# Gyeeta/gyeeta

Hardware: AMD Instinct MI355X
Metric: events/sec ingested + p50/p99 quantile error vs reference, 1→8 MI355X (higher is better)
Workload: dtype int64; 1 GPU; C3/C4: 10000 hosts x 1000 services, raw 24-B tcp_ipv4_resp_event_t stream, uniform over services, 1 window (ingest + window close) per step; service_keys_total=10000000, multi_level_windows=0, td_pend_cap=1920, td_pend_cap_is_library_default=False, exchange=none, exchange_requested=none, exchange_fallback=False

## Files before the change

### gyeeta_amd/csrc/gys_engine.hip

```cpp
#include <hip/hip_runtime.h>

#include <algorithm>
#include <array>
#include <atomic>
#include <chrono>
#include <cmath>
#include <cstdarg>
#include <cstdio>
#include <cstdlib>
#include <cstring>
#include <deque>
#include <functional>
#include <map>
#include <memory>
#include <set>
#include <string>
#include <thread>
#include <condition_variable>
#include <mutex>
#include <unordered_map>
#include <unordered_set>
#include <vector>

#include <dlfcn.h>
// ... 663 lines not shown
		fin.list[FIN_CLASS2] = c->merge_list2;
		fin.list[FIN_HUGE] = c->huge_list;
		fin.counts = c->merge_count;
		fin.td_run = c->td_run;
		fin.svc_host = c->svc_host;
		fin.host_spill = c->host_spill;
		fin.counters = c->counters;
		fin.staged_cap = (uint32_t)std::min<uint64_t>(c->staged.cap, 0xFFFFFFFFull);
	}
	if (b.td && c->prespill) {
		fin.td_run0 = c->td_run0;
		fin.td_run1 = c->td_run1;
		fin.td_prevm = c->td_prevm;
		fin.hot = c->pre_hot;
		fin.hot_wr = b.pre ? ((c->pre_seq & 1u) ^ 1u) : (c->pre_seq & 1u);
		fin.append_list = c->append_list;
		fin.append_cap = (uint32_t)c->append_list.cap;
		fin.td_pend = c->td_pend;
		fin.staged = c->staged;
		HIPCHK(hipMemsetAsync(c->merge_count + FIN_APPEND, 0, (FIN_NWORDS - FIN_APPEND) * 4, c->stream));
	}
	if (!b.front.host_local) return GYS_OK;
	RespHostP &hp = b.hp;
	hp.ev = (const uint64_t *)b.d_ev;
	hp.n = b.n;
	hp.segs = b.slot->segs.dev;
	hp.nsegs = b.nsegs;
	hp.hdesc = c->hdesc;
	hp.htbl = c->htbl;
	hp.hlst = c->hlst;
	hp.cand = c->cand_pool;
	hp.hll32 = c->hll32;
	hp.td_cur = c->td_cur;
	hp.td_pend = c->td_pend;
	hp.pcap = c->pcap;
	hp.td_run = c->td_run;
	hp.td_run1 = c->td_run1;
	hp.run_delta = (long long)(((intptr_t)c->staged.p - (intptr_t)c->td_pend.p) / 4);
	hp.staged = c->staged;
	hp.host_spill = c->host_spill;
	hp.spill_stamp = ++c->spill_stamp;
	fin.spill_stamp = hp.spill_stamp;
	hp.fin = fin;
	static const uint32_t dbg = [] { const char *e = getenv("GYS_DBG"); return e ? (uint32_t)atoi(e) : 0u; }();
	hp.dbg = dbg;
	hp.counters = c->counters;
	hp.svc_hll = c->svc_hll;
	hp.svc_hll_p = c->cfg.svc_hll_p;
	hp.ghist = (unsigned long long *)(c->arena + c->al.off_i64sum) + c->al.i64_ghist;
	hp.gmax = (long long *)(c->arena + c->al.off_i64max);
	hp.lds_tbl_entries = b.front.max_tbl;
	hp.lds_key_entries = (uint32_t)align_up(b.front.max_l, 2);
	b.hgrid = b.nsegs;
	return GYS_OK;
}

template <bool SHARED, bool SPILL>
void launch_resp_host_tile(gys_ctx *c, const RespBatch &b)
{
	if (b.tile == 6144u) return launch_resp_host<12, SHARED, SPILL>(c, b.hgrid, b.dyn, b.hp);
	if (b.tile == 16384u) launch_resp_host<16, SHARED, SPILL>(c, b.hgrid, b.dyn, b.hp);
	else launch_resp_host<8, SHARED, SPILL>(c, b.hgrid, b.dyn, b.hp);
}

int resp_launch_host_local(gys_ctx *c, RespBatch &b)
{
	if (b.front.host_split || b.front.host_parts) {
		PinnedPair<gys_resp_seg> &vs = b.slot->vsegs;
		const uint64_t nv = resp_virtual_segments(c->resp_sv.data(), b.nsegs, b.front.host_split, c->cfg.max_hosts, nullptr);
		int rc = vs.grow(nv, (1u << 16) / sizeof(gys_resp_seg));
		if (rc) return rc;
		resp_virtual_segments(c->resp_sv.data(), b.nsegs, b.front.host_split, c->cfg.max_hosts, vs.host);
		HIPCHK(hipMemcpyAsync(vs.dev, vs.host, nv * sizeof(gys_resp_seg), hipMemcpyHostToDevice, c->stream));
		b.hp.segs = vs.dev;
		b.hp.nsegs = b.hgrid = (uint32_t)nv;
	}
	if (b.front.host_split) c->n_batches_host_split++;
	else c->n_batches_host_local++;
	if (b.pre) {
		ProfScope ps(c, "prespill");
		PreSpillP pp{};
		pp.td_cur = c->td_cur;
		pp.td_prevm = c->td_prevm;
		pp.td_run = c->td_run;
		pp.td_run0 = c->td_run0;
		pp.td_run1 = c->td_run1;
		pp.counts = c->merge_count;
		pp.hot = c->pre_hot;
		pp.hot_rd = c->pre_seq & 1u;
		pp.svc_host = c->svc_host;
		pp.host_batch = c->host_batch;
		pp.batch_stamp = c->batch_stamp;
		pp.nsvc = c->nsvc;
		pp.pcap = c->pcap;
		pp.pend_cap = c->pend_cap;
		pp.resv = (unsigned long long *)(c->merge_count + FIN_PRE_RESV);
		pp.run_limit = (uint32_t)std::min<uint64_t>(c->staged.cap - std::min<uint64_t>(b.n, c->staged.cap), 0xFFFFFFFFull);
		++c->pre_seq;
		hipLaunchKernelGGL(k_mark_hosts, dim3((b.nsegs + 255) / 256), dim3(256), 0, c->stream, b.slot->segs.dev, b.nsegs, c->host_batch, c->batch_stamp);
		hipLaunchKernelGGL(k_prespill, dim3((c->nsvc + 255) / 256), dim3(256), 0, c->stream, pp);
	}
	ProfScope ps(c, "resp_host");
	if (b.mode != 0) {
		if (b.front.host_split) launch_resp_host_mode<true, false>(c, b.mode, b.tile == 16384u, b.hgrid, b.dyn, b.hp);
		else launch_resp_host_mode<false, false>(c, b.mode, b.tile == 16384u, b.hgrid, b.dyn, b.hp);
	} else if (b.front.host_split) {
		launch_resp_host_tile<true, false>(c, b);
	} else {
		launch_resp_host_tile<false, false>(c, b);
	}
	return GYS_OK;
}

void resp_launch_pass1(gys_ctx *c, const RespBatch &b)
{
	c->n_batches_general++;
	RespP1 p{};
	p.ev = (const uint64_t *)b.d_ev;
	p.cand = c->cand_pool;
	p.n = b.n;
	p.segs = b.slot->segs.dev;
	p.nsegs = b.nsegs;
	p.lk = c->lk_tbl;
	p.svc_gid = c->svc_gid;
	p.hist_win = c->hist_win;
	p.bitmap = c->bitmap;
	p.hll32 = c->hll32;
	p.cms32 = (uint32_t *)(c->arena + c->al.off_u32) + c->al.u32_cms;
	p.batch_cnt = b.td ? c->batch_cnt : nullptr;
	p.ev_kv = b.td ? c->ev_kv : nullptr;
	p.counters = c->counters;
	p.svc_hll = c->svc_hll;
	p.svc_hll_p = c->cfg.svc_hll_p;
	p.ghist = (unsigned long long *)(c->arena + c->al.off_i64sum) + c->al.i64_ghist;
	p.gmax = (long long *)(c->arena + c->al.off_i64max);
	ProfScope ps(c, "resp_pass1");
	if (b.v6) hipLaunchKernelGGL(k_resp_pass1<true>, dim3(grid_for(b.n, 256, (uint32_t)c->ncu * 8)), dim3(256), 0, c->stream, p);
	else hipLaunchKernelGGL(k_resp_pass1<false>, dim3(grid_for(b.n, 256, (uint32_t)c->ncu * 8)), dim3(256), 0, c->stream, p);
}

void resp_launch_general(gys_ctx *c, const RespBatch &b)
{
	const uint32_t nsvc = c->nsvc, nblk = (nsvc + GYS_SCAN_TILE - 1) / GYS_SCAN_TILE;
	{
		ProfScope ps(c, "scan");
		hipLaunchKernelGGL(k_scan_block_sums, dim3(nblk), dim3(256), 0, c->stream, c->batch_cnt, nsvc, c->scan_block_sums);
		hipLaunchKernelGGL(k_scan_top, dim3(1), dim3(256), 0, c->stream, c->scan_block_sums, nblk);
		hipLaunchKernelGGL(k_scan_final, dim3(nblk), dim3(256), 0, c->stream, c->batch_cnt, nsvc, c->scan_block_sums, c->batch_off);
	}
	{
		ProfScope ps(c, "scatter");
		hipLaunchKernelGGL(k_resp_scatter, dim3(grid_for(b.n, 256, (uint32_t)c->ncu * 8)), dim3(256), 0, c->stream, c->ev_kv, b.n, c->batch_off, c->staged);
	}
	ProfScope ps(c, "key_append");
	AppendP ap{};
	ap.batch_cnt = c->batch_cnt;
	ap.off_end = c->batch_off;
	ap.staged = c->staged;
	ap.td_cur = c->td_cur;
	ap.td_pend = c->td_pend;
	ap.pcap = c->pcap;
	ap.nsvc = nsvc;
	const uint32_t nchunks = (nsvc + 63u) / 64u;
	hipLaunchKernelGGL(k_key_append, dim3(std::min<uint32_t>((nchunks + 3u) / 4u, (uint32_t)c->ncu * 8)), dim3(256), 0, c->stream, ap);
}

void resp_launch_finalize(gys_ctx *c, RespBatch &b)
{
	const bool host_local = b.front.host_local;
	if (!host_local || b.front.host_split) {
		ProfScope ps(c, "key_finalize");
		b.fin.batch_off = host_local ? nullptr : c->batch_off;
		hipLaunchKernelGGL(k_key_finalize, dim3((c->nsvc + 255) / 256), dim3(256), 0, c->stream, b.fin);
	}
	if (b.pre)
		hipLaunchKernelGGL(k_run_append, dim3((uint32_t)c->ncu), dim3(256), 0, c->stream, c->append_list, c->merge_count + FIN_APPEND, c->staged, c->td_pend, c->pcap);
	if (host_local && b.n > (uint64_t)c->pcap - c->pend_cap) {
		ProfScope ps(c, "resp_spill");
		if (b.mode != 0) launch_resp_host_mode<true, true>(c, b.mode, b.tile == 16384u, b.hgrid, b.dyn, b.hp);
		else launch_resp_host_tile<true, true>(c, b);
	}
}

void resp_launch_slow_pass(gys_ctx *c, const DigestP &d, uint32_t cap, int top)
{
	MergeP mp{};
	mp.d = d;
	mp.list = c->merge_list_slow;
	mp.count = c->merge_count + FIN_SLOW;
	const dim3 grid(std::max(1u, std::min<uint32_t>(cap, (uint32_t)c->ncu)));
	if (top == 2) hipLaunchKernelGGL((k_digest_merge<GYS_MERGE_LDS_MAX, 1024u>), grid, dim3(1024), 0, c->stream, mp);
	else if (top == 0 && c->merge_fast <= GYS_MERGE_CLASS0) hipLaunchKernelGGL((k_digest_merge<GYS_MERGE_CLASS0, 256u>), grid, dim3(256), 0, c->stream, mp);
	else hipLaunchKernelGGL((k_digest_merge<GYS_MERGE_CLASS1, 256u>), grid, dim3(256), 0, c->stream, mp);
}

void resp_launch_merges(gys_ctx *c, const RespBatch &b)
{
	const uint32_t nsvc = c->nsvc, ncu = (uint32_t)c->ncu;
	const uint32_t cap = (uint32_t)std::min<uint64_t>(nsvc, b.n);
	const bool reach[3] = {true, c->merge_fast < GYS_MERGE_CLASS1 && b.n > c->merge_fast - c->pend_cap, b.n > GYS_MERGE_CLASS1 - c->pend_cap};
	const int top = reach[2] ? 2 : reach[1] ? 1 : 0;
	MergeEnt *const lists[3] = {c->merge_list, c->merge_list1, c->merge_list2};
	MergeBP bp{};
	bp.d = digest_params(c);
	bp.slow_list = c->merge_list_slow;
	bp.slow_count = c->merge_count + FIN_SLOW;
	for (int cls = 0; cls < 3; ++cls) {
		if (!reach[cls]) continue;
		ProfScope ps(c, cls ? "digest_merge_big" : "digest_merge");
		bp.list = lists[cls];
		bp.count = c->merge_count + FIN_CLASS0 + cls;
		if (cls == 0) {
			const dim3 bgrid(std::max(1u, std::min<uint32_t>(cap, ncu * 8)));
			if (c->merge_fast <= 1024u) hipLaunchKernelGGL((k_digest_bins<false, 4u>), bgrid, dim3(256), 0, c->stream, bp);
			else if (c->merge_fast <= 2048u) hipLaunchKernelGGL((k_digest_bins<false, 8u>), bgrid, dim3(256), 0, c->stream, bp);
			else hipLaunchKernelGGL((k_digest_bins<false, 16u>), bgrid, dim3(256), 0, c->stream, bp);
		} else if (cls == 1) {
			hipLaunchKernelGGL((k_digest_bins<false, 16u>), dim3(std::max(1u, std::min<uint32_t>(cap, ncu * GYS_MB_WAVES16))), dim3(256), 0, c->stream, bp);
		} else {
			const uint32_t cap2 = (uint32_t)std::min<uint64_t>(nsvc, b.n / (GYS_MERGE_CLASS1 - c->pend_cap) + 1);
			hipLaunchKernelGGL((k_digest_bins<false, 64u>), dim3(std::max(1u, std::min<uint32_t>(cap2, ncu * 8))), dim3(256), 0, c->stream, bp);
		}
		if (cls == top) resp_launch_slow_pass(c, bp.d, cap, top);
	}
}

void resp_launch_huge(gys_ctx *c, const RespBatch &b)
{
	ProfScope ps(c, "digest_huge");
	Huge2P q{};
	q.d = digest_params(c);
// ... 3161 lines not shown
} GYS_CATCH_ALL

int gys_export_svc_counters(gys_ctx *c, uint32_t first_slot, uint32_t nslots, uint64_t *out)
try {
	GYS_ENTER(c);
	RANGE_CHECK(first_slot, nslots);
	{
		const int rcf = conn_fold(c);
		if (rcf) return rcf;
	}
	HIPCHK(hipMemcpyAsync(out, c->svc_ctr + (size_t)first_slot * 4, (size_t)nslots * 32, hipMemcpyDeviceToHost, c->stream));
	HIPCHK(hipStreamSynchronize(c->stream));
	return GYS_OK;
} GYS_CATCH_ALL

int gys_export_svc_hll(gys_ctx *c, uint32_t first_slot, uint32_t nslots, uint8_t *out)
try {
	GYS_ENTER(c);
	RANGE_CHECK(first_slot, nslots);
	if (!c->svc_hll) return GYS_ERR_STATE;
	HIPCHK(hipMemcpyAsync(out, c->svc_hll + ((size_t)first_slot << c->cfg.svc_hll_p), (size_t)nslots << c->cfg.svc_hll_p, hipMemcpyDeviceToHost, c->stream));
	HIPCHK(hipStreamSynchronize(c->stream));
	return GYS_OK;
} GYS_CATCH_ALL

int gys_export_svc_hll_level(gys_ctx *c, int level, uint64_t tusec, uint32_t first_slot, uint32_t nslots, uint8_t *out)
try {
	GYS_ENTER(c);
	RANGE_CHECK(first_slot, nslots);
	HLL_LEVEL_CHECK(level);
	if (!nslots) return GYS_OK;
	DevBuf<uint8_t> tmp;
	int rc = tmp.grow((size_t)nslots << c->cfg.svc_hll_p, c->stream);
	if (rc == GYS_OK) rc = hll_level_view(c, level, tusec, first_slot, nslots, tmp.p, nullptr);
	if (rc) return rc;
	HIPCHK(hipMemcpyAsync(out, tmp.p, (size_t)nslots << c->cfg.svc_hll_p, hipMemcpyDeviceToHost, c->stream));
	HIPCHK(hipStreamSynchronize(c->stream));
	return GYS_OK;
} GYS_CATCH_ALL

int gys_get_counters(gys_ctx *c, gys_counters *out)
try {
	GYS_ENTER(c);
	if (!c || !out) return GYS_ERR_INVAL;
	uint64_t v[32];
	static_assert(CTR_NUM <= 31, "counter block (the last word is the sink of k_read_events)");
	HIPCHK(hipMemcpyAsync(v, c->counters, sizeof(v), hipMemcpyDeviceToHost, c->stream));
	HIPCHK(hipStreamSynchronize(c->stream));
#ifdef GYS_RESP_TIMING
	{
		unsigned long long t[16];
		HIPCHK(hipMemcpyFromSymbol(t, HIP_SYMBOL(gys::g_resp_timing), sizeof(t)));
		unsigned long long tot = 0;
		for (int i = 0; i < 12; ++i) tot += t[i];
		static const char *nm[12] = {"loads", "probe2", "probe3+", "kept/atomics", "ghist+hash", "hllq/store", "barrier1", "scan1+b", "scan2+b", "image+b", "prologue", "flush"};
		fprintf(stderr, "GYS_RESP_TIMING waves %llu ticks %llu:", t[15], tot);
		for (int i = 0; i < 12; ++i) fprintf(stderr, " %s %.1f%%", nm[i], tot ? 100.0 * (double)t[i] / (double)tot : 0.0);
		fprintf(stderr, "\n");
	}
#endif
#ifdef GYS_HUGE_TIMING
	fprintf(stderr, "GYS_HUGE_TIMING ticks: load %llu words+tail %llu scan %llu assign %llu writeback %llu | entries %llu npend %llu nc %llu\n", (unsigned long long)v[20], (unsigned long long)v[21], (unsigned long long)v[22], (unsigned long long)v[23], (unsigned long long)v[24], (unsigned long long)v[25], (unsigned long long)v[26], (unsigned long long)v[27]);
#endif
	out->resp_events = v[CTR_RESP_EVENTS];
	out->resp_dropped_range = v[CTR_RESP_DROP_RANGE];
	out->resp_dropped_nolistener = v[CTR_RESP_DROP_NOLISTENER];
	out->conn_events = v[CTR_CONN_EVENTS];
	out->conn_unknown_service = v[CTR_CONN_UNKNOWN];
	out->conn_new = v[CTR_CONN_NEW];
	out->conn_closed = v[CTR_CONN_CLOSED];
	out->conn_closed_no_notify = v[CTR_CONN_CLOSED_NO_NOTIFY];
	out->conn_client_side = v[CTR_CONN_CLI_SIDE];
	out->resp_run_overflow = v[CTR_RESP_RUN_OVERFLOW];
	out->lstate_records = v[CTR_LSTATE_RECORDS];
	out->lstate_missed = v[CTR_LSTATE_MISSED];
	out->lstate_errors = v[CTR_LSTATE_ERRORS];
	out->lstate_deleted = v[CTR_LSTATE_DELETED];
	out->resp_batches_host_local = c->n_batches_host_local;
	out->resp_batches_general = c->n_batches_general;
	out->window_graph_launches = c->win_graph_launches;
	out->resp_batches_host_split = c->n_batches_host_split;
	out->td_merges = v[CTR_TD_MERGES];
	out->td_merge_values = v[CTR_TD_MERGE_VALUES];
	out->actconn_records = v[CTR_ACTCONN_RECORDS];
	out->actconn_remote_listen = v[CTR_ACTCONN_REMOTE_LISTEN];
	out->actconn_unknown_listener = v[CTR_ACTCONN_UNKNOWN];
	out->stage_waits = c->ring.waits.load();
	auto snap = [](SubQ &q, uint64_t *calls, uint64_t *submissions) {
		std::lock_guard<std::mutex> g(q.mu);
		*calls = q.calls;
		*submissions = q.submissions;
		return q.tail_flushes;
	};
	out->resp_tail_flushes = snap(c->sq[SubQ::RESP], &out->resp_calls_queued, &out->resp_submissions);
	out->rec_tail_flushes = snap(c->sq[SubQ::CONN], &out->conn_calls_queued, &out->conn_submissions);
	out->rec_tail_flushes += snap(c->sq[SubQ::LSTATE], &out->lstate_calls_queued, &out->lstate_submissions);
	return GYS_OK;
} GYS_CATCH_ALL

int gys_resp_queue_pending(gys_ctx *c, uint64_t *events)
try {
	if (!c || !events) return GYS_ERR_INVAL;
	SubQ &q = c->sq[SubQ::RESP];
	std::lock_guard<std::mutex> g(q.mu);
	uint64_t n = 0;
	if (q.open >= 0) n += q.b[q.open].fill;
	for (int bi : q.sealed) n += q.b[bi].fill;
	*events = n;
	return GYS_OK;
} GYS_CATCH_ALL

// ... 374 lines not shown
```

### gyeeta_amd/csrc/gys_kernels.hpp

```cpp
#pragma once

#include "gys_device.hpp"

namespace gys {

#define GYS_HUGE_VALUE_BITS 20
#define GYS_HUGE_BINS (1u << GYS_HUGE_VALUE_BITS)
#define GYS_ROW_BITS 6
#define GYS_ROW_MASK 0x3Fu
#define GYS_ROW_V6 0x20u
#define GYS_BM_WORDS 32u
#define GYS_STAGED_WORD(tresp, cli_port) ((uint64_t)(((uint32_t)(tresp) << GYS_ROW_BITS) | ((uint32_t)(cli_port) & 0x1Fu)))
#define GYS_STAGED_WORD_FAM(tresp, cli_port, v6) ((uint32_t)(((uint32_t)(tresp) << GYS_ROW_BITS) | ((v6) ? GYS_ROW_V6 : 0u) | ((uint32_t)(cli_port) & 0x1Fu)))

enum { CTR_RESP_EVENTS = 0, CTR_RESP_DROP_RANGE, CTR_RESP_DROP_NOLISTENER, CTR_CONN_EVENTS, CTR_CONN_UNKNOWN, CTR_LSTATE_RECORDS,
       CTR_LSTATE_MISSED, CTR_LSTATE_ERRORS, CTR_LSTATE_DELETED, CTR_TD_MERGES, CTR_TD_MERGE_VALUES, CTR_ACTCONN_RECORDS, CTR_ACTCONN_REMOTE_LISTEN, CTR_ACTCONN_UNKNOWN,
       CTR_CONN_NEW, CTR_CONN_CLOSED, CTR_CONN_CLOSED_NO_NOTIFY, CTR_CONN_CLI_SIDE, CTR_RESP_RUN_OVERFLOW, CTR_NUM };

__global__ void k_table_set(DevTable t, const uint64_t *kv, uint32_t n)
{
	const uint32_t i = blockIdx.x * blockDim.x + threadIdx.x;
	if (i >= n) return;
	const uint64_t key = kv[2u * i];
	uint32_t h = get_uint64_hash(key) & t.mask;
// ... 313 lines not shown
	const uint64_t stride = (uint64_t)gridDim.x * blockDim.x;
	for (uint64_t i = (uint64_t)blockIdx.x * blockDim.x + threadIdx.x; i < n; i += stride) {
		const uint64_t kv = ev_kv[i];
		if (kv == ~0ull) continue;
		const uint32_t pos = atomicAdd(&off[(uint32_t)(kv >> 32)], 1u);
		staged[pos] = (uint32_t)kv;
	}
}

struct TdMeta {
	uint32_t npend;
	uint16_t nh;
	uint16_t nw;
	uint32_t win_epoch;
	uint32_t hw_epoch;
};
static_assert(sizeof(TdMeta) == 16, "TdMeta is read and written as one 16-byte word");
static_assert(GYS_TD_PEND_CAP == GYS_TDIGEST_PEND_CAP, "gysketch.h and gys_tdigest_tbl.h disagree on the t-digest buffer size");
static_assert(GYS_TD_NB == GYS_TDIGEST_NB && GYS_TD_NB <= 256, "the merge kernels hold one cluster per thread of a 256-thread group");

#define GYS_SPILL_BIT 0x80000000u
#define GYS_RESPILL_BIT 0x40000000u
#define GYS_MERGE_LDS_MAX 16384u
#define GYS_PCAP_MAX 16384u

struct MergeEnt {
	uint32_t slot;
	uint32_t nbuf;
	uint32_t mrun;
	uint32_t off_end;
};

__global__ void k_minmax_init(int2 *mm, uint64_t n)
{
	for (uint64_t i = (uint64_t)blockIdx.x * blockDim.x + threadIdx.x; i < n; i += (uint64_t)gridDim.x * blockDim.x) mm[i] = make_int2(INT32_MAX, INT32_MIN);
}

#define GYS_MERGE_CLASS0 1024u
#define GYS_MERGE_CLASS1 4096u
static_assert(GYS_TDIGEST_MERGE_FAST == GYS_MERGE_CLASS0, "the early re-clustering rule keeps a key's merges inside merge size class 0 (default buffer size)");
enum {
	FIN_CLASS0 = 0, FIN_CLASS1, FIN_CLASS2,
	FIN_HUGE,
	FIN_RUN_ALLOC,
	FIN_SLOW,
	FIN_HUGE_FB,
	FIN_HUGE_NENT,
	FIN_BATCH_CLEARED,
	FIN_QUERY_ONE = FIN_BATCH_CLEARED,
	FIN_HUGE_TAIL,
	FIN_HUGE_TB,
	FIN_APPEND = 12,
	FIN_PRE_RESV = 14,
	FIN_NWORDS = 16
};

struct FinP {
	uint32_t *td_cur;
	TdMeta *td_meta;
	uint32_t nsvc, pcap, epoch;
	uint32_t pend_cap, merge_fast;
	uint32_t *resp_win;
	MergeEnt *list[4];
	uint32_t *counts;
	uint32_t *td_run;
	const uint32_t *batch_off;
	const uint32_t *svc_host;
	uint32_t *host_spill;
	uint32_t spill_stamp;
	uint64_t *counters;
	const uint32_t *td_run0, *td_run1;
	uint32_t *td_prevm, *hot;
	uint32_t hot_wr;
	MergeEnt *append_list;
	uint32_t class2_max;
	uint32_t append_cap;
	uint32_t staged_cap;
	uint32_t *td_pend;
	const uint32_t *staged;
};

template <bool WRITE_CUR>
__device__ __forceinline__ int finalize_one(const FinP &p, bool valid, uint32_t key, uint32_t cur, MergeEnt &ent)
{
	int cls = -1;
	ent = MergeEnt{};
	if (valid) {
		const uint4 mraw = *(const uint4 *)&p.td_meta[key];
		const uint32_t npend0 = mraw.x;
		const bool pre = (cur & GYS_SPILL_BIT) != 0u;
		uint32_t run0 = 0;
		bool run_ok = false;
		if (pre) {
			run0 = p.td_run0[key];
			const uint32_t fill = p.td_run[key];
			run_ok = fill <= p.td_run1[key];
			cur = npend0 + (fill - run0);
			if (fill == run0) {
				p.td_cur[key] = npend0;
				p.td_prevm[key] = 0u;
			}
		}
		if (cur != npend0) {
			const uint32_t m = cur - npend0;
			uint32_t nh = mraw.y & 0xFFFFu, nw = mraw.y >> 16, win_epoch = mraw.z;
			if (win_epoch != p.epoch) {
				nw = npend0;
// ... 259 lines not shown
}

struct HostDesc {
	uint32_t tbl_off;
	uint32_t mask;
	uint32_t nlst;
	uint32_t lst_off;
	uint32_t part;
	uint32_t pmask;
	uint32_t cand_off;
	uint32_t pad;
};

#define GYS_HOST_TBL_EMPTY 0xFFFFFFFFFFFFFFFFull
#define GYS_EV_DROPPED 0xFFFFFFFFu
#define GYS_HOST_THREADS 1024
#define GYS_RESP_THREADS(TPT) ((TPT) == 12 ? 512 : 1024)
#define GYS_SPLIT_PART 65536u

#ifdef GYS_RESP_TIMING
__device__ unsigned long long g_resp_timing[16];
#define GYS_TICK(i) do { const unsigned long long t_now__ = (unsigned long long)clock64(); tacc[i] += (uint32_t)(t_now__ - t_prev__); t_prev__ = t_now__; } while (0)
#else
#define GYS_TICK(i) do { } while (0)
#endif
struct RespHostP {
	const uint64_t *ev;
	uint64_t n;
	const gys_resp_seg *segs;
	uint32_t nsegs;
	const HostDesc *hdesc;
	const uint64_t *htbl;
	const uint32_t *hlst;
	const ListenerCand *cand;
	uint32_t *hll32;
	uint32_t *td_cur;
	uint32_t *td_pend;
	uint32_t pcap;
	uint32_t *td_run;
	const uint32_t *td_run1;
	long long run_delta;
	uint32_t *staged;
	const uint32_t *host_spill;
	uint32_t spill_stamp;
	uint64_t *counters;
	uint8_t *svc_hll;
	uint32_t svc_hll_p;
	unsigned long long *ghist;
	long long *gmax;
	uint32_t lds_tbl_entries;
	uint32_t lds_key_entries;
	FinP fin;
	uint32_t dbg;
};

__host__ __device__ __forceinline__ size_t resp_host_lds_bytes(uint32_t tbl_entries, uint32_t key_entries, uint32_t tile)
{
	return ((size_t)tbl_entries + 2u) * 8u + (size_t)key_entries * 24u + ((size_t)tile + 2u) * 6u;
}

#ifndef GYS_RESP_DBG
#define GYS_RESP_DBG 0
#endif
#define GYS_GH_STRIDE 17u
#define GYS_HQ_CAP 512u
#define GYS_DST_BIAS 65536ull
#ifndef GYS_OPAQUE_LOADED4
#define GYS_OPAQUE_LOADED4(a) asm volatile("" : "+v"(a[0]), "+v"(a[1]), "+v"(a[2]), "+v"(a[3]))
#endif
#define GYS_MEM_FENCE() asm volatile("" ::: "memory")

template <uint32_t T>
__host__ __device__ __forceinline__ uint32_t resp_slot_stride(uint32_t r)
{
	return r >= 4u * T ? T : (((r + 3u) / 4u + 63u) & ~63u);
}

template <int TPT, bool SHARED, bool SPILL, bool SVCHLL, int MODE = 0>
__global__ __launch_bounds__(GYS_RESP_THREADS(TPT), 4) void k_resp_host(RespHostP p_arg)
{
#if defined(__HIP_DEVICE_COMPILE__)
	typedef const RespHostP __attribute__((address_space(4))) *KernargP;
	KernargP p_k = (KernargP)__builtin_amdgcn_kernarg_segment_ptr();
#define GYS_RESP_P_RELOAD() asm volatile("" : "+s"(p_k))
	const RespHostP &p = *(const RespHostP *)p_k;
#else
#define GYS_RESP_P_RELOAD() (void)0
	const RespHostP &p = p_arg;
#endif
	constexpr uint32_t T = GYS_RESP_THREADS(TPT);
	constexpr uint32_t TILE = (uint32_t)TPT * T;
	constexpr bool DBG = GYS_RESP_DBG != 0;
	constexpr bool V6 = MODE == 2;
	constexpr uint32_t SW = V6 ? GYS_EV6_WORDS : 3u;
	GYS_DYN_LDS(uint64_t, s_dyn);
	__shared__ uint32_t s_wsum[T / 64];
	__shared__ uint32_t s_drop[2];
	__shared__ uint32_t s_floor[2];
	__shared__ uint32_t s_fqm[4];
	__shared__ unsigned long long s_gh[16 * GYS_GH_STRIDE];
	__shared__ int32_t s_gmax;
	__shared__ uint32_t s_bk[256];
	__shared__ uint32_t s_hq[SPILL ? 1 : GYS_HQ_CAP];
	__shared__ uint32_t s_hqn;
	__shared__ FinWg s_fin;
	__shared__ uint32_t s_park[64];
	if (!SPILL) resp_bucket_lut_init(s_bk, threadIdx.x, T);
	const uint32_t Lc = p.lds_key_entries;
	uint64_t *s_tbl = s_dyn;
	uint64_t *s_dst = s_dyn + p.lds_tbl_entries + 2u;
	uint32_t *s_cur = (uint32_t *)(s_dst + Lc);
	uint32_t *s_slot = s_cur + Lc;
	uint32_t *s_ts2 = s_slot + Lc;
	uint32_t *s_val = s_ts2 + 2u * Lc;
	uint16_t *s_key = (uint16_t *)(s_val + TILE + 2u);
	const uint32_t tid = threadIdx.x, lane = tid & 63u, wave = tid >> 6;
	const gys_resp_seg seg = p.segs[blockIdx.x];
	const uint64_t e0 = seg.first_event;
	uint32_t nx = blockIdx.x + 1;
	if (seg.reserved)
		while (nx < p.nsegs && p.segs[nx].reserved && p.segs[nx].host_slot == seg.host_slot && p.segs[nx].first_event == e0) ++nx;
	uint64_t e1 = nx < p.nsegs ? p.segs[nx].first_event : p.n;
	if (e1 > p.n) e1 = p.n;
	if (e1 <= e0) return;
	if (SPILL && p.host_spill[seg.host_slot] != p.spill_stamp) return;
	const HostDesc hd = p.hdesc[seg.reserved ? seg.reserved - 1u : seg.host_slot];
	const uint32_t mask = hd.mask, L = hd.nlst;
	for (uint32_t i = tid; i <= mask; i += T) s_tbl[i] = p.htbl[hd.tbl_off + i];
	for (uint32_t k = tid; k < L; k += T) {
		const uint32_t slot = p.hlst[hd.lst_off + k];
		const uint32_t c = p.td_cur[slot];
		s_slot[k] = slot;
		s_cur[k] = SPILL ? (c & GYS_RESPILL_BIT) : c;
		s_ts2[k] = 0;
		s_ts2[Lc + k] = 0;
	}
	if (tid < 2) s_drop[tid] = 0;
	if (tid < 16u * GYS_GH_STRIDE) s_gh[tid] = 0;
	if (tid == 0) {
		s_hqn = 0;
		s_floor[0] = SPILL ? 0u : 0xFFFFFFFFu;
		s_floor[1] = 0xFFFFFFFFu;
		s_gmax = INT32_MIN;
		s_tbl[mask + 1u] = p.htbl[hd.tbl_off];
		s_val[TILE] = 0;
		s_key[TILE] = 0;
	}
	__syncthreads();
	if (!SPILL) {
		if (e1 - e0 >= 4096u) {
			uint32_t mn = 0xFFFFFFFFu;
			const uint4 *h4 = (const uint4 *)p.hll32;
			for (uint32_t i = tid; i < (1u << GYS_HLL_P) / 4u; i += T) {
				const uint4 v = h4[i];
				mn = min(min(mn, min(v.x, v.y)), min(v.z, v.w));
			}
			mn = wave_min_u32(mn);
			if (lane == 0) atomicMin(&s_floor[0], mn);
		} else if (tid == 0) {
			s_floor[0] = 0;
		}
		__syncthreads();
		if (tid == 0) s_floor[1] = s_floor[0];
		if (tid < 4) s_fqm[tid] = s_floor[0];
	}
	uint32_t hll_floor = 0;
	const uint32_t K = (L + T - 1) / T;
	const uint32_t klo = min(L, tid * K), khi = min(L, klo + K);
	uint32_t *const dst = SPILL ? p.staged : p.td_pend;
	uint32_t *const dstb = dst - GYS_DST_BIAS;

	uint32_t ndrop_range = 0, ndrop_nol = 0, tile_no = 0, dbg_sink = 0;
#ifdef GYS_RESP_TIMING
	uint32_t tacc[16] = {0, 0, 0, 0, 0, 0, 0, 0, 0, 0, 0, 0, 0, 0, 0, 0};
	unsigned long long t_prev__ = (unsigned long long)clock64();
#endif
	const uint32_t tid24 = 24u * tid;
	const uint32_t wbase = (uint32_t)__builtin_amdgcn_readfirstlane((int)(tid & ~63u));
	int32_t tmax = INT32_MIN, wmax = -1;
	GYS_TICK(10);
	for (uint64_t t0 = e0; t0 < e1; t0 += TILE, ++tile_no) {
		GYS_RESP_P_RELOAD();
		uint32_t *const s_ts = s_ts2 + (tile_no & 1u) * Lc;
#if GYS_PARK_INDEX
#if defined(__HIP_DEVICE_COMPILE__)
		typedef uint32_t park_ix_t;
#else
		typedef ptrdiff_t park_ix_t;
#endif
		const park_ix_t park_ix = (park_ix_t)(&s_park[lane] - s_ts);
#endif
		if (!SPILL) hll_floor = (uint32_t)__builtin_amdgcn_readfirstlane((int)s_floor[tile_no & 1u]);
		const uint64_t left = e1 - t0;
		const uint32_t rem = (uint32_t)__builtin_amdgcn_readfirstlane((int)(left < (uint64_t)TILE ? (uint32_t)left : TILE));
		const uint64_t *const tb = p.ev + (uint64_t)SW * t0;
		uint32_t wd[TPT], lr[TPT];
#pragma unroll
		for (int u = 0; u < TPT; ++u) {
			wd[u] = GYS_EV_DROPPED;
			lr[u] = 0;
		}
#pragma unroll 1
		for (int g = 0; g < TPT; g += 4) {
			if ((uint32_t)g * T >= rem) break;
			const uint32_t S = resp_slot_stride<T>(rem - (uint32_t)g * T);
			if (wbase >= S) break;
			uint64_t w0[4], w1[4], w2[4];
			bool in[4];
#pragma unroll
			for (int u = 0; u < 4; ++u) {
				const uint32_t first = (uint32_t)g * T + (uint32_t)u * S, last = min(rem, first + S);
				const uint32_t ob_raw = tid24 + 24u * first;
				in[u] = ob_raw < 24u * last;
				const uint32_t ob = in[u] ? ob_raw : 0u;
				if (V6) {
					static_assert(GYS_EV6_WORDS == 6, "ob = 24 o: word 6 o of the tile is ob / 4");
					w0[u] = 0;
					w1[u] = tb[ob / 4u + 4u];
					w2[u] = tb[ob / 4u + 5u];
				} else {
					const char *const tbb = (const char *)tb;
					w0[u] = *(const uint64_t *)(tbb + ob);
					w1[u] = *(const uint64_t *)(tbb + ob + 8u);
					w2[u] = *(const uint64_t *)(tbb + ob + 16u);
				}
			}
			GYS_OPAQUE_LOADED4(w0);
			GYS_OPAQUE_LOADED4(w1);
			GYS_OPAQUE_LOADED4(w2);
			GYS_TICK(0);
			uint32_t tresp[4], local[4];
			uint64_t ea[4], eb[4];
// ... 294 lines not shown
				s_key[pos] = (uint16_t)(lr[u] & 0xFFFu);
			}
		}
		__syncthreads();
		GYS_TICK(9);
		if (!SPILL && hq_cur < (hq_e >> 16)) atomicMax(&p.hll32[hq_e & 0xFFFFu], hq_e >> 16);
		{
			uint32_t ntile = 0;
#pragma unroll
			for (uint32_t w = 0; w < T / 64; ++w) ntile += s_wsum[w];
			if (DBG && (p.dbg & 3u)) ntile = 0;
			constexpr int FU = 8;
			constexpr uint32_t NQ = (1u << GYS_HLL_P) / 16u / T;
			uint4 fq[NQ];
			const bool fq_on = !SPILL && t0 + 2ull * TILE < e1;
			if (fq_on) {
#pragma unroll
				for (uint32_t j = 0; j < NQ; ++j) fq[j] = ((const uint4 *)p.hll32)[(tile_no & 3u) * ((1u << GYS_HLL_P) / 16u) + j * T + tid];
			}
			for (uint32_t eb0 = 0; eb0 < ntile; eb0 += (uint32_t)FU * T) {
				uint32_t kk[FU], vv[FU];
				uint64_t dd[FU];
#pragma unroll
				for (int j = 0; j < FU; ++j) {
					const uint32_t e = eb0 + (uint32_t)j * T + tid;
					const uint32_t ee = e < ntile ? e : TILE;
					kk[j] = s_key[ee];
					vv[j] = s_val[ee];
				}
				GYS_MEM_FENCE();
#pragma unroll
				for (int j = 0; j < FU; ++j) dd[j] = s_dst[kk[j]];
				GYS_MEM_FENCE();
#pragma unroll
				for (int j = 0; j < FU; ++j) {
					const uint32_t e = eb0 + (uint32_t)j * T + tid;
					if (e < ntile && dd[j]) dstb[dd[j] + e] = vv[j];
				}
			}
			if (fq_on) {
				uint32_t mn = 0xFFFFFFFFu;
#pragma unroll
				for (uint32_t j = 0; j < NQ; ++j) mn = min(min(mn, min(fq[j].x, fq[j].y)), min(fq[j].z, fq[j].w));
				mn = wave_min_u32(mn);
				if (lane == 0) {
					const uint32_t qn = tile_no & 3u;
					atomicMin(&s_fqm[qn], mn);
					atomicMin(&s_floor[tile_no & 1u], min(min(mn, s_fqm[(qn + 1u) & 3u]), min(s_fqm[(qn + 2u) & 3u], s_fqm[(qn + 3u) & 3u])));
				}
			}
		}
		GYS_TICK(11);
	}
#ifdef GYS_RESP_TIMING
	if (!SPILL && lane == 0) {
#pragma unroll
		for (int i = 0; i < 12; ++i) atomicAdd(&g_resp_timing[i], (unsigned long long)tacc[i]);
		atomicAdd(&g_resp_timing[15], 1ull);
	}
#endif
	if (SPILL) return;
	if (DBG && dbg_sink == 0xDEADBEEFu) p.counters[CTR_RESP_EVENTS] = 1;
	if (wmax >= 0) tmax = wmax >> GYS_ROW_BITS;
	tmax = wave_max_i32(tmax);
	if (lane == 0 && tmax != INT32_MIN) atomicMax(&s_gmax, tmax);
	if (ndrop_range) atomicAdd(&s_drop[0], ndrop_range);
	if (ndrop_nol) atomicAdd(&s_drop[1], ndrop_nol);
	__syncthreads();
	if (tid < 64u) {
		unsigned long long cnt = 0, sum = 0;
		if (tid < 15u) {
			for (uint32_t w = 0; w < 16u; ++w) {
				const unsigned long long v = s_gh[w * GYS_GH_STRIDE + tid];
				cnt += v >> 40;
				sum += v & ((1ull << 40) - 1);
			}
			if (cnt) {
				atomicAdd(&p.ghist[2 * tid], cnt);
				atomicAdd(&p.ghist[2 * tid + 1], sum);
			}
		}
		unsigned long long tot = cnt;
#pragma unroll
		for (int d = 8; d >= 1; d >>= 1) tot += (unsigned long long)__shfl_xor((long long)tot, d, 64);
		if (tid == 0 && tot) atomicAdd(&p.ghist[30], tot);
	}
	if (!SHARED) {
		constexpr int KMAX = (int)(2048u / T);
		bool fvalid[KMAX];
		uint32_t fkey[KMAX], fcur[KMAX];
#pragma unroll
		for (int j = 0; j < KMAX; ++j) {
			const uint32_t k = (uint32_t)j * T + tid;
			fvalid[j] = k < L;
			fkey[j] = fvalid[j] ? s_slot[k] : 0u;
			fcur[j] = fvalid[j] ? s_cur[k] : 0u;
		}
		finalize_keys_wg<true, KMAX>(p.fin, &s_fin, tid, lane, fvalid, fkey, fcur);
	}
	if (tid == 0) {
		if (s_gmax != INT32_MIN) atomicMax(p.gmax, (long long)s_gmax);
		if (hd.part == 0u) atomicAdd((unsigned long long *)&p.counters[CTR_RESP_EVENTS], (unsigned long long)(e1 - e0));
		if (s_drop[0]) atomicAdd((unsigned long long *)&p.counters[CTR_RESP_DROP_RANGE], (unsigned long long)s_drop[0]);
		if (s_drop[1]) atomicAdd((unsigned long long *)&p.counters[CTR_RESP_DROP_NOLISTENER], (unsigned long long)s_drop[1]);
	}
}

struct AppendP {
	uint32_t *batch_cnt;
	const uint32_t *off_end;
	const uint32_t *staged;
	uint32_t *td_cur;
	uint32_t *td_pend;
	uint32_t pcap, nsvc;
};

__global__ __launch_bounds__(256) void k_key_append(AppendP p)
{
	const uint32_t lane = threadIdx.x & 63u;
	const uint32_t nchunks = (p.nsvc + 63u) / 64u, nwaves = gridDim.x * 4u;
	for (uint32_t chunk = blockIdx.x * 4u + (threadIdx.x >> 6); chunk < nchunks; chunk += nwaves) {
		const uint32_t key = chunk * 64u + lane;
		const uint32_t m = key < p.nsvc ? p.batch_cnt[key] : 0u;
		unsigned long long todo = __ballot(m != 0);
		if (!todo) continue;
		const uint32_t oend = m ? p.off_end[key] : 0u;
		const uint32_t cur = m ? p.td_cur[key] : 0u;
		if (m) {
			p.batch_cnt[key] = 0;
			p.td_cur[key] = cur + m;
		}
		while (todo) {
			const int k = __ffsll((long long)todo) - 1;
			todo &= todo - 1;
			const uint32_t km = (uint32_t)__shfl((int)m, k, 64), ke = (uint32_t)__shfl((int)oend, k, 64), kc = (uint32_t)__shfl((int)cur, k, 64);
			if ((uint64_t)kc + km > (uint64_t)p.pcap) continue;
			const uint32_t *src = p.staged + (ke - km);
			uint32_t *dst = p.td_pend + (size_t)(chunk * 64u + (uint32_t)k) * p.pcap + kc;
			for (uint32_t i = lane; i < km; i += 64u) dst[i] = src[i];
		}
	}
}

struct DigestP {
	int64_t *td_sum;
	uint32_t *td_cnt;
	TdMeta *td_meta;
	int2 *td_minmax;
	uint32_t *td_pend;
	uint32_t *td_cur;
	uint32_t pcap, nsvc;
	uint32_t pend_cap;
	const uint32_t *staged;
	gys_hist_rec *hist_win, *hist_all;
	uint32_t *bitmap;
};

#define GYS_WAVE_SYNC()                                              \
// ... 2907 lines not shown
```

Before: 76.89 billion events/s.

## Convert resp_host kernel to a persistent grid with an atomic segment work queue

The per-host response kernel now launches at most one workgroup per CU (two for the 6144 tile). Each workgroup loops over segments, taking the next one from an atomic counter that is cleared before launch. Per-workgroup setup (LDS stats, drop counters, ghist, gmax) and the final flush to global counters run once per workgroup rather than once per segment. The HLL floor scan is also cached across segments. This removes launch and prologue/epilogue cost for very many small segments, but fewer resident workgroups may lower occupancy, and the stale HLL floor plus reliance on the counter reset add risk. The spill pass keeps the old one-workgroup-per-segment grid.

```diff
diff --git a/gyeeta_amd/csrc/gys_engine.hip b/gyeeta_amd/csrc/gys_engine.hip
--- a/gyeeta_amd/csrc/gys_engine.hip
+++ b/gyeeta_amd/csrc/gys_engine.hip
@@ -739,7 +739,14 @@
 	hp.lds_tbl_entries = b.front.max_tbl;
 	hp.lds_key_entries = (uint32_t)align_up(b.front.max_l, 2);
 	b.hgrid = b.nsegs;
-	return GYS_OK;
+	if (!c->prespill) HIPCHK(hipMemsetAsync(c->merge_count + FIN_RESP_WORK, 0, 4, c->stream));
+	return GYS_OK;
+}
+
+void resp_persistent_grid(gys_ctx *c, RespBatch &b)
+{
+	b.hgrid = std::min<uint32_t>(b.hp.nsegs, (uint32_t)c->ncu * (b.tile == 6144u ? 2u : 1u));
+	b.hp.work = c->merge_count + FIN_RESP_WORK;
 }
 
 template <bool SHARED, bool SPILL>
@@ -787,6 +794,7 @@
 		hipLaunchKernelGGL(k_mark_hosts, dim3((b.nsegs + 255) / 256), dim3(256), 0, c->stream, b.slot->segs.dev, b.nsegs, c->host_batch, c->batch_stamp);
 		hipLaunchKernelGGL(k_prespill, dim3((c->nsvc + 255) / 256), dim3(256), 0, c->stream, pp);
 	}
+	resp_persistent_grid(c, b);
 	ProfScope ps(c, "resp_host");
 	if (b.mode != 0) {
 		if (b.front.host_split) launch_resp_host_mode<true, false>(c, b.mode, b.tile == 16384u, b.hgrid, b.dyn, b.hp);
@@ -864,6 +872,8 @@
 		hipLaunchKernelGGL(k_run_append, dim3((uint32_t)c->ncu), dim3(256), 0, c->stream, c->append_list, c->merge_count + FIN_APPEND, c->staged, c->td_pend, c->pcap);
 	if (host_local && b.n > (uint64_t)c->pcap - c->pend_cap) {
 		ProfScope ps(c, "resp_spill");
+		b.hgrid = b.hp.nsegs;
+		b.hp.work = nullptr;
 		if (b.mode != 0) launch_resp_host_mode<true, true>(c, b.mode, b.tile == 16384u, b.hgrid, b.dyn, b.hp);
 		else launch_resp_host_tile<true, true>(c, b);
 	}
@@ -4131,11 +4141,11 @@
 		unsigned long long t[16];
 		HIPCHK(hipMemcpyFromSymbol(t, HIP_SYMBOL(gys::g_resp_timing), sizeof(t)));
 		unsigned long long tot = 0;
-		for (int i = 0; i < 12; ++i) tot += t[i];
-		static const char *nm[12] = {"loads", "probe2", "probe3+", "kept/atomics", "ghist+hash", "hllq/store", "barrier1", "scan1+b", "scan2+b", "image+b", "prologue", "flush"};
+		for (int i = 0; i < 13; ++i) tot += t[i];
+		static const char *nm[13] = {"loads", "probe2", "probe3+", "kept/atomics", "ghist+hash", "hllq/store", "barrier1", "scan1+b", "scan2+b", "image+b", "prologue", "flush", "epilogue"};
 		fprintf(stderr, "GYS_RESP_TIMING waves %llu ticks %llu:", t[15], tot);
-		for (int i = 0; i < 12; ++i) fprintf(stderr, " %s %.1f%%", nm[i], tot ? 100.0 * (double)t[i] / (double)tot : 0.0);
-		fprintf(stderr, "\n");
+		for (int i = 0; i < 13; ++i) fprintf(stderr, " %s %.1f%%", nm[i], tot ? 100.0 * (double)t[i] / (double)tot : 0.0);
+		fprintf(stderr, " | workgroups %llu resident %.3f ms in all (ncu %d)\n", t[14], (double)t[13] / 1e5, c->ncu);
 	}
 #endif
 #ifdef GYS_HUGE_TIMING
diff --git a/gyeeta_amd/csrc/gys_kernels.hpp b/gyeeta_amd/csrc/gys_kernels.hpp
--- a/gyeeta_amd/csrc/gys_kernels.hpp
+++ b/gyeeta_amd/csrc/gys_kernels.hpp
@@ -389,7 +389,8 @@
 	FIN_HUGE_TB,
 	FIN_APPEND = 12,
 	FIN_PRE_RESV = 14,
-	FIN_NWORDS = 16
+	FIN_RESP_WORK = 16,
+	FIN_NWORDS = 17
 };
 
 struct FinP {
@@ -755,6 +756,7 @@
 	uint32_t lds_key_entries;
 	FinP fin;
 	uint32_t dbg;
+	uint32_t *work;
 };
 
 __host__ __device__ __forceinline__ size_t resp_host_lds_bytes(uint32_t tbl_entries, uint32_t key_entries, uint32_t tile)
@@ -785,7 +787,7 @@
 #if defined(__HIP_DEVICE_COMPILE__)
 	typedef const RespHostP __attribute__((address_space(4))) *KernargP;
 	KernargP p_k = (KernargP)__builtin_amdgcn_kernarg_segment_ptr();
-#define GYS_RESP_P_RELOAD() asm volatile("" : "+s"(p_k))
+#define GYS_RESP_P_RELOAD() do { p_k = (KernargP)__builtin_amdgcn_kernarg_segment_ptr(); asm volatile("" : "+s"(p_k)); } while (0)
 	const RespHostP &p = *(const RespHostP *)p_k;
 #else
 #define GYS_RESP_P_RELOAD() (void)0
@@ -808,6 +810,14 @@
 	__shared__ uint32_t s_hqn;
 	__shared__ FinWg s_fin;
 	__shared__ uint32_t s_park[64];
+	__shared__ uint32_t s_next;
+	__shared__ uint32_t s_fl_ok;
+	__shared__ unsigned long long s_nev;
+#ifdef GYS_RESP_TIMING
+	const unsigned long long wg_t0__ = (unsigned long long)wall_clock64();
+	uint32_t tacc[16] = {0, 0, 0, 0, 0, 0, 0, 0, 0, 0, 0, 0, 0, 0, 0, 0};
+	unsigned long long t_prev__ = (unsigned long long)clock64();
+#endif
 	if (!SPILL) resp_bucket_lut_init(s_bk, threadIdx.x, T);
 	const uint32_t Lc = p.lds_key_entries;
 	uint64_t *s_tbl = s_dyn;
@@ -818,19 +828,44 @@
 	uint32_t *s_val = s_ts2 + 2u * Lc;
 	uint16_t *s_key = (uint16_t *)(s_val + TILE + 2u);
 	const uint32_t tid = threadIdx.x, lane = tid & 63u, wave = tid >> 6;
-	const gys_resp_seg seg = p.segs[blockIdx.x];
+	if (tid < 2) s_drop[tid] = 0;
+	if (tid < 16u * GYS_GH_STRIDE) s_gh[tid] = 0;
+	if (tid == 0) {
+		s_gmax = INT32_MIN;
+		s_fl_ok = 0;
+		s_nev = 0;
+	}
+	uint32_t hll_floor = 0;
+	uint32_t *const dst = SPILL ? p.staged : p.td_pend;
+	uint32_t *const dstb = dst - GYS_DST_BIAS;
+	uint32_t ndrop_range = 0, ndrop_nol = 0, tile_no = 0, dbg_sink = 0;
+	const uint32_t tid24 = 24u * tid;
+	const uint32_t wbase = (uint32_t)__builtin_amdgcn_readfirstlane((int)(tid & ~63u));
+	int32_t tmax = INT32_MIN, wmax = -1;
+	uint32_t sg = blockIdx.x;
+	while (sg < p.nsegs) {
+	uint32_t ptid = tid;
+	GYS_OPAQUE_VGPR(ptid);
+	uint32_t nxt = 0;
+	if (ptid == 0) nxt = p.work ? gridDim.x + atomicAdd(p.work, 1u) : sg + gridDim.x;
+	const gys_resp_seg seg = p.segs[sg];
 	const uint64_t e0 = seg.first_event;
-	uint32_t nx = blockIdx.x + 1;
+	uint32_t nx = sg + 1;
 	if (seg.reserved)
 		while (nx < p.nsegs && p.segs[nx].reserved && p.segs[nx].host_slot == seg.host_slot && p.segs[nx].first_event == e0) ++nx;
 	uint64_t e1 = nx < p.nsegs ? p.segs[nx].first_event : p.n;
 	if (e1 > p.n) e1 = p.n;
-	if (e1 <= e0) return;
-	if (SPILL && p.host_spill[seg.host_slot] != p.spill_stamp) return;
+	if (e1 <= e0 || (SPILL && p.host_spill[seg.host_slot] != p.spill_stamp)) {
+		__syncthreads();
+		if (ptid == 0) s_next = nxt;
+		__syncthreads();
+		sg = (uint32_t)__builtin_amdgcn_readfirstlane((int)s_next);
+		continue;
+	}
 	const HostDesc hd = p.hdesc[seg.reserved ? seg.reserved - 1u : seg.host_slot];
 	const uint32_t mask = hd.mask, L = hd.nlst;
-	for (uint32_t i = tid; i <= mask; i += T) s_tbl[i] = p.htbl[hd.tbl_off + i];
-	for (uint32_t k = tid; k < L; k += T) {
+	for (uint32_t i = ptid; i <= mask; i += T) s_tbl[i] = p.htbl[hd.tbl_off + i];
+	for (uint32_t k = ptid; k < L; k += T) {
 		const uint32_t slot = p.hlst[hd.lst_off + k];
 		const uint32_t c = p.td_cur[slot];
 		s_slot[k] = slot;
@@ -838,49 +873,44 @@
 		s_ts2[k] = 0;
 		s_ts2[Lc + k] = 0;
 	}
-	if (tid < 2) s_drop[tid] = 0;
-	if (tid < 16u * GYS_GH_STRIDE) s_gh[tid] = 0;
-	if (tid == 0) {
+	if (ptid == 0) {
 		s_hqn = 0;
-		s_floor[0] = SPILL ? 0u : 0xFFFFFFFFu;
-		s_floor[1] = 0xFFFFFFFFu;
-		s_gmax = INT32_MIN;
+		if (SPILL || !s_fl_ok) {
+			s_floor[0] = SPILL ? 0u : 0xFFFFFFFFu;
+			s_floor[1] = 0xFFFFFFFFu;
+		}
 		s_tbl[mask + 1u] = p.htbl[hd.tbl_off];
 		s_val[TILE] = 0;
 		s_key[TILE] = 0;
 	}
 	__syncthreads();
-	if (!SPILL) {
+	if (ptid == 0) {
+		s_next = nxt;
+		if (!SPILL && hd.part == 0u) s_nev += e1 - e0;
+	}
+	if (!SPILL && !__builtin_amdgcn_readfirstlane((int)s_fl_ok)) {
 		if (e1 - e0 >= 4096u) {
 			uint32_t mn = 0xFFFFFFFFu;
 			const uint4 *h4 = (const uint4 *)p.hll32;
-			for (uint32_t i = tid; i < (1u << GYS_HLL_P) / 4u; i += T) {
+			for (uint32_t i = ptid; i < (1u << GYS_HLL_P) / 4u; i += T) {
 				const uint4 v = h4[i];
 				mn = min(min(mn, min(v.x, v.y)), min(v.z, v.w));
 			}
 			mn = wave_min_u32(mn);
-			if (lane == 0) atomicMin(&s_floor[0], mn);
-		} else if (tid == 0) {
+			if ((ptid & 63u) == 0) {
+				atomicMin(&s_floor[0], mn);
+				atomicMin(&s_floor[1], mn);
+			}
+		} else if (ptid == 0) {
 			s_floor[0] = 0;
+			s_floor[1] = 0;
 		}
 		__syncthreads();
-		if (tid == 0) s_floor[1] = s_floor[0];
-		if (tid < 4) s_fqm[tid] = s_floor[0];
-	}
-	uint32_t hll_floor = 0;
+		if (ptid < 4) s_fqm[ptid] = s_floor[0];
+		if (ptid == 0 && e1 - e0 >= 4096u) s_fl_ok = 1;
+	}
 	const uint32_t K = (L + T - 1) / T;
 	const uint32_t klo = min(L, tid * K), khi = min(L, klo + K);
-	uint32_t *const dst = SPILL ? p.staged : p.td_pend;
-	uint32_t *const dstb = dst - GYS_DST_BIAS;
-
-	uint32_t ndrop_range = 0, ndrop_nol = 0, tile_no = 0, dbg_sink = 0;
-#ifdef GYS_RESP_TIMING
-	uint32_t tacc[16] = {0, 0, 0, 0, 0, 0, 0, 0, 0, 0, 0, 0, 0, 0, 0, 0};
-	unsigned long long t_prev__ = (unsigned long long)clock64();
-#endif
-	const uint32_t tid24 = 24u * tid;
-	const uint32_t wbase = (uint32_t)__builtin_amdgcn_readfirstlane((int)(tid & ~63u));
-	int32_t tmax = INT32_MIN, wmax = -1;
 	GYS_TICK(10);
 	for (uint64_t t0 = e0; t0 < e1; t0 += TILE, ++tile_no) {
 		GYS_RESP_P_RELOAD();
@@ -1281,15 +1311,29 @@
 		}
 		GYS_TICK(11);
 	}
-#ifdef GYS_RESP_TIMING
-	if (!SPILL && lane == 0) {
-#pragma unroll
-		for (int i = 0; i < 12; ++i) atomicAdd(&g_resp_timing[i], (unsigned long long)tacc[i]);
-		atomicAdd(&g_resp_timing[15], 1ull);
-	}
-#endif
-	if (SPILL) return;
-	if (DBG && dbg_sink == 0xDEADBEEFu) p.counters[CTR_RESP_EVENTS] = 1;
+	if (!SHARED && !SPILL) {
+		constexpr int KMAX = (int)(2048u / T);
+		bool fvalid[KMAX];
+		uint32_t fkey[KMAX], fcur[KMAX];
+		uint32_t etid = tid;
+		GYS_OPAQUE_VGPR(etid);
+#pragma unroll
+		for (int j = 0; j < KMAX; ++j) {
+			const uint32_t k = (uint32_t)j * T + etid;
+			fvalid[j] = k < L;
+			fkey[j] = fvalid[j] ? s_slot[k] : 0u;
+			fcur[j] = fvalid[j] ? s_cur[k] : 0u;
+		}
+		finalize_keys_wg<true, KMAX>(p.fin, &s_fin, etid, etid & 63u, fvalid, fkey, fcur);
+	} else {
+		__syncthreads();
+	}
+	sg = (uint32_t)__builtin_amdgcn_readfirstlane((int)s_next);
+	GYS_TICK(12);
+	}
+	if (!SPILL && DBG && dbg_sink == 0xDEADBEEFu) p.counters[CTR_RESP_EVENTS] = 1;
+	if (!SPILL) {
+	if (wmax >= 0) tmax = wmax >> GYS_ROW_BITS;
 	if (wmax >= 0) tmax = wmax >> GYS_ROW_BITS;
 	tmax = wave_max_i32(tmax);
 	if (lane == 0 && tmax != INT32_MIN) atomicMax(&s_gmax, tmax);
@@ -1314,25 +1358,25 @@
 		for (int d = 8; d >= 1; d >>= 1) tot += (unsigned long long)__shfl_xor((long long)tot, d, 64);
 		if (tid == 0 && tot) atomicAdd(&p.ghist[30], tot);
 	}
-	if (!SHARED) {
-		constexpr int KMAX = (int)(2048u / T);
-		bool fvalid[KMAX];
-		uint32_t fkey[KMAX], fcur[KMAX];
-#pragma unroll
-		for (int j = 0; j < KMAX; ++j) {
-			const uint32_t k = (uint32_t)j * T + tid;
-			fvalid[j] = k < L;
-			fkey[j] = fvalid[j] ? s_slot[k] : 0u;
-			fcur[j] = fvalid[j] ? s_cur[k] : 0u;
-		}
-		finalize_keys_wg<true, KMAX>(p.fin, &s_fin, tid, lane, fvalid, fkey, fcur);
-	}
 	if (tid == 0) {
 		if (s_gmax != INT32_MIN) atomicMax(p.gmax, (long long)s_gmax);
-		if (hd.part == 0u) atomicAdd((unsigned long long *)&p.counters[CTR_RESP_EVENTS], (unsigned long long)(e1 - e0));
+		if (s_nev) atomicAdd((unsigned long long *)&p.counters[CTR_RESP_EVENTS], s_nev);
 		if (s_drop[0]) atomicAdd((unsigned long long *)&p.counters[CTR_RESP_DROP_RANGE], (unsigned long long)s_drop[0]);
 		if (s_drop[1]) atomicAdd((unsigned long long *)&p.counters[CTR_RESP_DROP_NOLISTENER], (unsigned long long)s_drop[1]);
 	}
+	}
+#ifdef GYS_RESP_TIMING
+	GYS_TICK(12);
+	if (!SPILL && lane == 0) {
+#pragma unroll
+		for (int i = 0; i < 13; ++i) atomicAdd(&g_resp_timing[i], (unsigned long long)tacc[i]);
+		atomicAdd(&g_resp_timing[15], 1ull);
+	}
+	if (!SPILL && tid == 0) {
+		atomicAdd(&g_resp_timing[13], (unsigned long long)wall_clock64() - wg_t0__);
+		atomicAdd(&g_resp_timing[14], 1ull);
+	}
+#endif
 }
 
 struct AppendP {
```

Result: slower. 63.22 billion events/s (-17.8%).
